# yesint/molar

Measured on AMD Instinct MI355X. Metric: frames/sec + Matom-pairs/sec, 1M-atom PBC neighbor search + RMSD fit, higher is better.
Workload: dtype f32; 1 GPU; 1M-atom synthetic triclinic box A, per frame: PBC neighbour search rc=1.2 nm (ordered pair list in HBM) + Kabsch RMSD fit/COM/gyration of a 100k-atom selection; natoms=1000000, selection_atoms=100000, frames_per_gpu=1451, parallelism=frames sharded over 1 rank(s), no data-path collective, streams_per_gpu=2, measure_overlapped_with_search=True

## Files before the change

molar_amd/csrc/pair_kernels.hpp:

```cpp
#pragma once

#include "boxmath.hpp"
#include "common.hpp"

namespace mh {
namespace pairk {

enum { MODE_COUNT = 0, MODE_FILL = 1, MODE_HIST = 2 };

#ifndef MH_COUNT_WPE
#define MH_COUNT_WPE 6
#endif
#ifndef MH_FILL_WPE
#define MH_FILL_WPE 8
#endif
#ifndef MH_WPB
#define MH_WPB 1
#endif
constexpr int waves_per_block(int mode) { return mode == MODE_HIST ? 4 : MH_WPB; }
constexpr int KREG = 8;
constexpr int FIFO_CAP = 128;
#ifndef MOLAR_HIP_NO_WIDE_FLUSH
#define MOLAR_HIP_WIDE_FLUSH 1
#endif
constexpr int FIFO_WIDE = 256;
constexpr uint32_t XCD_RUN = 128;
constexpr float F32_EPS = 1.1920929e-07f;
constexpr bool MASKED_COUNT_SORTED = true;

static __constant__ uint8_t MASKS[14][6] = {
    {0, 0, 0, 0, 0, 0},
    {0, 0, 0, 1, 0, 0}, {0, 0, 0, 0, 1, 0}, {0, 0, 0, 0, 0, 1},
    {0, 0, 0, 1, 1, 0}, {0, 0, 0, 1, 0, 1}, {0, 0, 0, 0, 1, 1},
    {0, 0, 0, 1, 1, 1},
    {1, 0, 0, 0, 1, 0}, {1, 0, 0, 0, 0, 1}, {0, 1, 0, 0, 0, 1},
    {1, 1, 0, 0, 0, 1}, {1, 0, 1, 0, 1, 0}, {0, 1, 1, 1, 0, 0},
};


typedef float v4f_t __attribute__((ext_vector_type(4)));
__device__ __forceinline__ float4 gload4(const float4 *p, size_t i) {
    const v4f_t v = ((const __attribute__((address_space(1))) v4f_t *)p)[i];
    return make_float4(v.x, v.y, v.z, v.w);
}
__device__ __forceinline__ uint32_t gload_u32(const uint32_t *p, size_t i) {
    return ((const __attribute__((address_space(1))) uint32_t *)p)[i];
}
__device__ __forceinline__ void gstore_u32(uint32_t *p, size_t i, uint32_t v) {
    ((__attribute__((address_space(1))) uint32_t *)p)[i] = v;
}
__device__ __forceinline__ float uniform_f32(float v) { return __uint_as_float(__builtin_amdgcn_readfirstlane(__float_as_uint(v))); }
__device__ __forceinline__ float4 lload4(const float4 *p, uint32_t i) {
    const v4f_t v = ((const __attribute__((address_space(3))) v4f_t *)p)[i];
    return make_float4(v.x, v.y, v.z, v.w);
}

struct SearchParams {
    const float4 *sa;
    const float4 *sb;
    const uint32_t *csa;
    const uint32_t *csb;
    const float *vdwa;
    const float *vdwb;
    const float4 *aabb_b;
    const float4 *perm_b;
    const float4 *chunk_aabb_b;
    const uint4 *h16_b;
    const float4 *cell_org_b;
    uint32_t mfma_count;
    const struct TaskDesc *task_desc;
    uint32_t *maskbuf;
    const unsigned long long *task_moff;
    unsigned long long mask_cap_units;
    unsigned long long out_cap;
    uint32_t dx, dy, dz;
    uint32_t pbc;
    uint32_t use_box;
    uint32_t nblocks;
    uint32_t wrap_kind;
    uint32_t prune_wrapped;
    float prune_limit2;
    uint32_t approx_wrapped;
    float band_lo, band_hi;
    uint32_t hist_nbins;
    float hist_min, hist_max;
    unsigned long long *hist_bins;
    unsigned long long *hist_total;
    const float *hist_edges;
    float hist_scale;
    uint32_t hist_lean;
    const uint32_t *hist_nslots;
#ifdef MOLAR_HIP_DEBUG_KNOBS
    uint32_t debug_skip;
    unsigned long long *dbg;
#endif
    float cutoff2;
    uint64_t ntasks;
    molar_hip_box box;
    alignas(16) float shifts4[96];
    uint32_t hist_big;
};

struct TaskDesc {
    uint32_t a0, n1, b0, n2, cb, flags, pad0, pad1;
};

struct SlotDesc {
    uint32_t a0, n1, b0, n2;
// ... 120 lines not shown
    if (WK == WK_DIAG) {
        sx = M[0] * fx;
        sy = M[4] * fy;
        sz = M[8] * fz;
    } else if (WK == WK_UPPER) {
        sx = (M[0] * fx + M[3] * fy) + M[6] * fz;
        sy = M[4] * fy + M[7] * fz;
        sz = M[8] * fz;
    } else {
        sx = (M[0] * fx + M[3] * fy) + M[6] * fz;
        sy = (M[1] * fx + M[4] * fy) + M[7] * fz;
        sz = (M[2] * fx + M[5] * fy) + M[8] * fz;
    }
    v2f best2 = (sx * sx + sy * sy) + sz * sz;
    if (WK != WK_DIAG && B.nshift != 0 && wrap == MOLAR_HIP_PBC_FULL) {
        if (WIDE4) {
            for (int k = 0; k < B.nshift; k += 4) {
                float sh[12];
#pragma unroll
                for (int q = 0; q < 12; ++q) sh[q] = P.shifts4[3 * k + q];
#pragma unroll
                for (int q = 0; q < 4; ++q) {
                    const v2f cx = sx + sh[3 * q], cy = sy + sh[3 * q + 1], cz = sz + sh[3 * q + 2];
                    const v2f n2 = (cx * cx + cy * cy) + cz * cz;
                    best2.x = n2.x < best2.x ? n2.x : best2.x;
                    best2.y = n2.y < best2.y ? n2.y : best2.y;
                }
            }
        } else {
            for (int k = 0; k < B.nshift; ++k) {
                const v2f cx = sx + P.box.shifts[3 * k], cy = sy + P.box.shifts[3 * k + 1], cz = sz + P.box.shifts[3 * k + 2];
                const v2f n2 = (cx * cx + cy * cy) + cz * cz;
                best2.x = n2.x < best2.x ? n2.x : best2.x;
                best2.y = n2.y < best2.y ? n2.y : best2.y;
            }
        }
    }
    return best2;
}

struct Fifo {
    uint32_t *fi, *fj, *fd;
    uint32_t head, tail;
    uint32_t quota;
    uint64_t base;
    uint32_t room;
    bool has_pairs, has_dist;
    uint2 *pairs;
    float *dist;
    uint32_t *ids;
    uint32_t *hist;
    float hmin, hmax, hn;
    uint32_t recompute;
    const float4 *la;
    float4 *fq_store;
    float4 *fq;
    uint4 *lh;
    uint32_t wrap;
};

template <bool WIDE4 = false>
__device__ __forceinline__ float wrapped_d2_exact(const SearchParams &P, uint32_t wrap, float vx, float vy, float vz);

struct Hit {
    uint32_t i, j;
    float d2;
};
__device__ __forceinline__ Hit fifo_hit(const SearchParams &P, const Fifo &F, uint32_t s) {
    const uint32_t w = F.fd[s];
    if (F.recompute == 0u) return Hit{F.fi[s], F.fj[s], __uint_as_float(w)};
    float4 a, b;
    if (F.fq) {
        a = lload4(F.la, w);
        b = lload4(F.fq, s);
    } else {
        a = lload4(F.la, w >> 26);
        b = gload4(P.sb, w & 0x3FFFFFFu);
    }
    const float dx = b.x - a.x, dy = b.y - a.y, dz = b.z - a.z;
    const float d2 = F.recompute == 1u ? wrapped_d2_exact(P, F.wrap, dx, dy, dz) : (dx * dx + dy * dy) + dz * dz;
    return Hit{__float_as_uint(a.w), __float_as_uint(b.w), d2};
}

template <int KIND, int CAP = FIFO_CAP>
__device__ __forceinline__ void fifo_flush(const SearchParams &P, Fifo &F, uint32_t count, uint32_t lane) {
    if (lane < count && (F.hist || F.head + lane < F.room)) {
        const uint32_t s = (F.head + lane) & (CAP - 1);
        uint32_t pos = F.head;
#ifdef MOLAR_HIP_DEBUG_KNOBS
        if (P.debug_skip & 32u) pos &= 63u;
#endif
        if (KIND == MOLAR_HIP_SEARCH_WITHIN) {
            __builtin_nontemporal_store(F.fi[s], &F.ids[pos]);
        } else if (F.hist) {
            const float d = __builtin_sqrtf(fifo_hit(P, F, s).d2);
            float fb = __builtin_floorf(F.hn * (d - F.hmin) / (F.hmax - F.hmin));
            if (fb != fb) fb = 0.0f;
            if (fb >= 0.0f && fb < F.hn) atomicAdd(&F.hist[(uint32_t)fb], 1u);
        } else {
            const Hit h = fifo_hit(P, F, s);
#ifdef MOLAR_HIP_DEBUG_KNOBS
            const float dist = __builtin_sqrtf(h.d2);
            const bool wr = (P.debug_skip & 16u) ? dist == -1.0f : true;
            if (F.has_pairs && wr) __builtin_nontemporal_store(((unsigned long long)h.j << 32) | h.i, reinterpret_cast<unsigned long long *>(&F.pairs[pos]));
            if (F.has_dist && wr) __builtin_nontemporal_store(dist, &F.dist[pos]);
#else
            if (F.has_pairs) __builtin_nontemporal_store(((unsigned long long)h.j << 32) | h.i, reinterpret_cast<unsigned long long *>(&F.pairs[pos]));
            if (F.has_dist) __builtin_nontemporal_store(__builtin_sqrtf(h.d2), &F.dist[pos]);
#endif
        }
    }
    F.head += count;
}

template <int KIND>
__device__ __forceinline__ void fifo_drain(const SearchParams &P, Fifo &F, uint32_t lane) {
    __builtin_amdgcn_wave_barrier();
    do {
        fifo_flush<KIND>(P, F, F.quota, lane);
        F.quota = 64u;
    } while (F.tail - F.head >= 64u);
}

template <int KIND>
__device__ __forceinline__ void fifo_flush_wide(const SearchParams &P, Fifo &F, uint32_t lane) {
    typedef uint32_t u4_t __attribute__((ext_vector_type(4)));
    typedef float f2_t __attribute__((ext_vector_type(2)));
    const uint32_t e = F.head + 2u * lane;
    if (e + 1u < F.room) {
        const uint32_t s0 = e & (FIFO_WIDE - 1), s1 = (e + 1u) & (FIFO_WIDE - 1);
        const u4_t pr = {F.fi[s0], F.fj[s0], F.fi[s1], F.fj[s1]};
        const f2_t ds = {__builtin_sqrtf(__uint_as_float(F.fd[s0])), __builtin_sqrtf(__uint_as_float(F.fd[s1]))};
        uint32_t at = F.head + lane;
        bool wr = true;
#ifdef MOLAR_HIP_DEBUG_KNOBS
        if (P.debug_skip & 16u) wr = ds.x == -1.0f;
        if (P.debug_skip & 32u) at = (F.head & 127u) + lane;
#endif
        if (F.has_pairs && wr) __builtin_nontemporal_store(pr, reinterpret_cast<u4_t *>(&F.pairs[at]));
        if (F.has_dist && wr) __builtin_nontemporal_store(ds, reinterpret_cast<f2_t *>(&F.dist[at]));
    } else if (e < F.room) {
        const uint32_t s0 = e & (FIFO_WIDE - 1);
        if (F.has_pairs) __builtin_nontemporal_store(((unsigned long long)F.fj[s0] << 32) | F.fi[s0], reinterpret_cast<unsigned long long *>(&F.pairs[F.head + lane]));
        if (F.has_dist) __builtin_nontemporal_store(__builtin_sqrtf(__uint_as_float(F.fd[s0])), &F.dist[F.head + lane]);
    }
    F.head += 128u;
}

template <int KIND>
__device__ __forceinline__ void fifo_drain_wide(const SearchParams &P, Fifo &F, uint32_t lane) {
    __builtin_amdgcn_wave_barrier();
    do {
        if (F.hist) {
            fifo_flush<KIND, FIFO_WIDE>(P, F, 64u, lane);
            fifo_flush<KIND, FIFO_WIDE>(P, F, 64u, lane);
        } else if (F.quota != 128u) {
            uint32_t left = F.quota;
            while (left) {
                const uint32_t c = left < 64u ? left : 64u;
                fifo_flush<KIND, FIFO_WIDE>(P, F, c, lane);
                left -= c;
            }
            F.quota = 128u;
        } else {
            fifo_flush_wide<KIND>(P, F, lane);
        }
    } while (F.tail - F.head >= 128u);
}

template <int KIND, bool FILL, int WK, bool TRI, int NCH, bool RUNTIME_NCH, bool WIDE4 = false>
__device__ __forceinline__ uint32_t run_task(const SearchParams &P, const Task &T, uint32_t i0, Fifo &F, uint32_t lane) {
    constexpr bool VDW = KIND == MOLAR_HIP_SEARCH_DOUBLE_VDW;
    constexpr bool WITHIN = KIND == MOLAR_HIP_SEARCH_WITHIN;
    constexpr bool STREAM = NCH == 0;
    constexpr int NPAIR = STREAM ? 1 : (NCH + 1) / 2;
    uint32_t total = 0;
    BoxRegs B;
    B.nshift = 0;
    if (WK != WK_NONE) {
#pragma unroll
        for (int k = 0; k < 9; ++k) {
            B.I[k] = P.box.inv[k];
            B.M[k] = P.box.m[k];
        }
        B.nshift = P.box.nshift;
    }
    const float cutoff2 = P.cutoff2;

    v2f bx[NPAIR], by[NPAIR], bz[NPAIR], bv[NPAIR];
    uint32_t bid[2 * NPAIR];
    auto load_b = [&](uint32_t jj, float &x, float &y, float &z, float &v, uint32_t &id) {
        float4 q = make_float4(0.f, 0.f, 0.f, 0.f);
        float rv = 0.f;
        if (jj < T.n2) {
            q = P.sb[T.b0 + jj];
            if (VDW) rv = P.vdwb[T.b0 + jj];
        }
        x = q.x; y = q.y; z = q.z; v = rv; id = __float_as_uint(q.w);
    };
    if (!STREAM) {
#pragma unroll
        for (int h = 0; h < NPAIR; ++h) {
            float x0, y0, z0, v0, x1, y1, z1, v1;
            load_b((uint32_t)(2 * h) * 64u + lane, x0, y0, z0, v0, bid[2 * h]);
            load_b((uint32_t)(2 * h + 1) * 64u + lane, x1, y1, z1, v1, bid[2 * h + 1]);
            bx[h] = v2f{x0, x1}; by[h] = v2f{y0, y1}; bz[h] = v2f{z0, z1}; bv[h] = v2f{v0, v1};
        }
    }
    const uint32_t nchunks = (T.n2 + 63u) >> 6;

    {
        float4 a = make_float4(0.f, 0.f, 0.f, 0.f);
        float ra = 0.f;
        if (i0 + lane < T.n1) {
            a = P.sa[T.a0 + i0 + lane];
            if (VDW) ra = P.vdwa[T.a0 + i0 + lane];
        }
        const uint32_t rows = T.n1 - i0 < T.rps ? T.n1 - i0 : T.rps;
        for (uint32_t r = 0; r < rows; ++r) {
            const uint32_t i = i0 + r;
            const float px = __int_as_float(__builtin_amdgcn_readlane(__float_as_int(a.x), r));
            const float py = __int_as_float(__builtin_amdgcn_readlane(__float_as_int(a.y), r));
            const float pz = __int_as_float(__builtin_amdgcn_readlane(__float_as_int(a.z), r));
            const uint32_t id_i = (uint32_t)__builtin_amdgcn_readlane(__float_as_int(a.w), r);
            float r1 = 0.f;
            if (VDW) r1 = __int_as_float(__builtin_amdgcn_readlane(__float_as_int(ra), r));
            bool found = false;
// ... 205 lines not shown

constexpr int MFMA_TILES = 10;

__device__ __forceinline__ float mfma_error_bound(float R, float c) {
    return 2.3841858e-07f * ((16.0f * R * R + 8.0f * c) + (4.0f * R + 1.0f));
}
__device__ __forceinline__ bool mfma_bound_usable(float R, float E, float c) {
    return R < 64.0f && E < 0.02f * c && (c + R * R) < 3.0e4f;
}

template <int KIND, bool TRI>
__device__ __forceinline__ uint32_t run_count_mfma(const SearchParams &P, const Task &T, uint32_t i0, float4 *la, uint4 *lh,
                                                   uint32_t lane, bool &done) {
    typedef uint32_t u4_t __attribute__((ext_vector_type(4)));
    typedef __attribute__((address_space(3))) u4_t lds_u4;
    typedef __attribute__((address_space(3))) uint32_t lds_u32;
    typedef __attribute__((address_space(1))) u4_t glb_u4;
    const float cutoff2 = P.cutoff2;
    const uint32_t rows = __builtin_amdgcn_readfirstlane(T.n1 - i0 < T.rps ? T.n1 - i0 : T.rps);
    const uint32_t kh = lane >> 5, cl = lane & 31u;
    const uint32_t nct = (T.n2 + 31u) >> 5;
    float4 a = make_float4(0.f, 0.f, 0.f, 0.f);
    if (lane < rows) a = gload4(P.sa, T.a0 + i0 + lane);
    const float4 org = gload4(P.cell_org_b, T.cb);
    bool need = lane < rows;
    if (!TRI) {
        const float4 blo = gload4(P.aabb_b, 2 * T.cb), bhi = gload4(P.aabb_b, 2 * T.cb + 1);
        need = need && !(aabb_d2(a.x, a.y, a.z, blo.x, blo.y, blo.z, bhi.x, bhi.y, bhi.z) > cutoff2);
    }
    const unsigned long long live = __builtin_amdgcn_ballot_w64(need);
    const uint32_t nlive = TRI ? rows : (uint32_t)__popcll(live);
    if (!TRI && nlive == 0u) return 0u;
    const uint32_t rank = TRI ? lane : __builtin_amdgcn_mbcnt_hi((uint32_t)(live >> 32), __builtin_amdgcn_mbcnt_lo((uint32_t)live, 0u));
    u4_t bq[MFMA_TILES];
#pragma unroll
    for (int t = 0; t < MFMA_TILES; ++t) {
        const uint32_t col = (uint32_t)t * 32u + cl;
        if (32u * (uint32_t)(t + 1) <= T.n2) {
            bq[t] = ((const glb_u4 *)P.h16_b)[T.b0 + col];
        } else {
            bq[t] = u4_t{0u, 0u, 0u, 0x00007BFFu};
            if (col < T.n2) bq[t] = ((const glb_u4 *)P.h16_b)[T.b0 + col];
        }
    }
    if (TRI || need) la[rank] = a;
    const float r0 = a.x - org.x, r1 = a.y - org.y, r2 = a.z - org.z;
    float ra2 = need ? (r0 * r0 + r1 * r1) + r2 * r2 : 0.0f;
    const bool fin = ra2 == ra2;
    for (int off = 32; off > 0; off >>= 1) ra2 = fmaxf(ra2, __shfl_xor(ra2, off, 64));
    const float R = 1.0001f * __builtin_sqrtf(ra2) + org.w;
    const float E = uniform_f32(mfma_error_bound(R, cutoff2));
    if (__builtin_amdgcn_ballot_w64(!fin) != 0ull || !mfma_bound_usable(R, E, cutoff2)) {
        done = false;
        return 0u;
    }
    {
        u4_t k0 = {0u, 0u, 0u, 0x00007BFFu}, k1 = {0u, 0u, 0u, 0x3C003C00u};
        if (!TRI) {
            ((lds_u4 *)lh)[2u * lane] = k0;
            ((lds_u4 *)lh)[2u * lane + 1u] = k1;
            __builtin_amdgcn_wave_barrier();
        }
        if (need) {
            const _Float16 h0 = (_Float16)r0, h1 = (_Float16)r1, h2 = (_Float16)r2;
            const _Float16 l0 = (_Float16)(r0 - (float)h0), l1 = (_Float16)(r1 - (float)h1), l2 = (_Float16)(r2 - (float)h2);
            const float e0 = (float)h0 + (float)l0, e1 = (float)h1 + (float)l1, e2 = (float)h2 + (float)l2;
            const float na = ((e0 * e0 + e1 * e1) + e2 * e2) - cutoff2;
            const _Float16 nh = (_Float16)na, nl = (_Float16)(na - (float)nh);
            const _Float16 m2 = (_Float16)-2.0f;
            const _Float16 g0 = m2 * h0, g1 = m2 * h1, g2 = m2 * h2, s0 = m2 * l0, s1 = m2 * l1, s2 = m2 * l2;
            k0 = u4_t{pack_h2(g0, g1), pack_h2(g2, g0), pack_h2(g1, g2), pack_h2(nh, nl)};
            k1 = u4_t{pack_h2(s0, s1), pack_h2(s2, s0), pack_h2(s1, s2), 0x3C003C00u};
        }
        if (TRI || need) {
            ((lds_u4 *)lh)[2u * rank] = k0;
            ((lds_u4 *)lh)[2u * rank + 1u] = k1;
        }
    }
    __builtin_amdgcn_wave_barrier();
    const u4_t a0q = ((const lds_u4 *)lh)[2u * cl + kh], a1q = ((const lds_u4 *)lh)[2u * (32u + cl) + kh];
    const v8h_t A0 = __builtin_bit_cast(v8h_t, a0q), A1 = __builtin_bit_cast(v8h_t, a1q);
    __builtin_amdgcn_wave_barrier();
    lds_u32 *todo = (lds_u32 *)lh;
    uint32_t ntodo = 0;
    uint32_t cnt = 0;
#pragma unroll
    for (int t = 0; t < MFMA_TILES; ++t) {
        if ((uint32_t)t < nct) {
            u4_t bt = bq[t];
            if (kh == 0u) bt.w = 0x3C003C00u;
            const v8h_t B = __builtin_bit_cast(v8h_t, bt);
#pragma unroll
            for (int rt = 0; rt < 2; ++rt) {
                bool diag = false;
                if (32u * (uint32_t)rt >= nlive) continue;
                if (TRI) {
                    const uint32_t row0 = i0 + 32u * (uint32_t)rt;
                    if (32u * (uint32_t)t + 31u <= row0) continue;
                    diag = 32u * (uint32_t)t <= row0 + 31u;
                }
                v16f_t acc = {0.f, 0.f, 0.f, 0.f, 0.f, 0.f, 0.f, 0.f, 0.f, 0.f, 0.f, 0.f, 0.f, 0.f, 0.f, 0.f};
                acc = __builtin_amdgcn_mfma_f32_32x32x16_f16(rt == 0 ? A0 : A1, B, acc, 0, 0, 0);
                if (TRI && diag) {
                    const int tv = (int)(32u * (uint32_t)t + cl) - (int)(i0 + 32u * (uint32_t)rt + 4u * kh);
#pragma unroll
                    for (int i = 0; i < 16; ++i) acc[i] = (tv > 8 * (i / 4) + (i % 4)) ? acc[i] : 1.0e30f;
                }
                uint32_t h = 0u;
                float m = INFINITY;
#pragma unroll
                for (int i = 0; i < 16; ++i) {
                    h = __builtin_amdgcn_alignbit(h, __float_as_uint(acc[i]), 31);
                    m = __builtin_fminf(m, __builtin_fabsf(acc[i]));
                }
                if (__builtin_amdgcn_ballot_w64(m < E) == 0ull) {
                    cnt += (uint32_t)__popc(h);
                } else {
                    if (lane == 0) todo[ntodo] = (uint32_t)(2 * t + rt);
                    ++ntodo;
                }
            }
        }
    }
    if (ntodo) {
        __builtin_amdgcn_wave_barrier();
        for (uint32_t q = 0; q < ntodo; ++q) {
            const uint32_t id = __builtin_amdgcn_readfirstlane(todo[q]);
            const uint32_t ct = id >> 1, rt = id & 1u;
            const uint32_t col = ct * 32u + cl;
            float4 b = make_float4(3.0e38f, 3.0e38f, 3.0e38f, 0.f);
            if (col < T.n2) b = gload4(P.sb, T.b0 + col);
            for (uint32_t r = 0; r < 16u; ++r) {
                const uint32_t row = 32u * rt + 16u * kh + r;
                const float4 p = lload4(la, row);
                const float dx = b.x - p.x, dy = b.y - p.y, dz = b.z - p.z;
                const float d2 = (dx * dx + dy * dy) + dz * dz;
                cnt += (row < nlive && (!TRI || col > i0 + row) && d2 <= cutoff2) ? 1u : 0u;
            }
        }
    }
    for (int off = 32; off > 0; off >>= 1) cnt += __shfl_xor(cnt, off, 64);
    return cnt;
}

template <int KIND>
__device__ __forceinline__ bool run_count_mfma_wrapped(const SearchParams &P, const Task &T, uint32_t i0, float4 *la, uint4 *lh,
                                                       uint32_t lane, uint32_t *mwords, uint32_t &count_out) {
    typedef uint32_t u4_t __attribute__((ext_vector_type(4)));
    typedef __attribute__((address_space(3))) u4_t lds_u4;
    typedef __attribute__((address_space(3))) uint32_t lds_u32;
    typedef __attribute__((address_space(1))) u4_t glb_u4;
    const float cutoff2 = P.cutoff2;
    const uint32_t rows = __builtin_amdgcn_readfirstlane(T.n1 - i0 < 64u ? T.n1 - i0 : 64u);
    const uint32_t kh = lane >> 5, cl = lane & 31u;
    const uint32_t nct = (T.n2 + 31u) >> 5, nch = (T.n2 + 63u) >> 6;
    float Sx = 0.f, Sy = 0.f, Sz = 0.f;
    for (int d = 0; d < 3; ++d) {
        if (!((T.wrap >> d) & 1u)) continue;
        const float sgn = ((T.wrap_b >> d) & 1u) ? 1.0f : -1.0f;
        Sx += sgn * P.box.m[3 * d];
        Sy += sgn * P.box.m[3 * d + 1];
        Sz += sgn * P.box.m[3 * d + 2];
    }
    float4 a = make_float4(0.f, 0.f, 0.f, 0.f);
    if (lane < rows) a = gload4(P.sa, T.a0 + i0 + lane);
    const float4 org = gload4(P.cell_org_b, T.cb);
    const float4 blo = gload4(P.aabb_b, 2 * T.cb), bhi = gload4(P.aabb_b, 2 * T.cb + 1);
    const bool need = lane < rows && !(aabb_d2(a.x - Sx, a.y - Sy, a.z - Sz, blo.x, blo.y, blo.z, bhi.x, bhi.y, bhi.z) > P.prune_limit2);
    const unsigned long long live = __builtin_amdgcn_ballot_w64(need);
    const uint32_t nlive = (uint32_t)__popcll(live);
    if (nlive == 0u) {
        count_out = 0u;
        return true;
    }
    const uint32_t rank = __builtin_amdgcn_mbcnt_hi((uint32_t)(live >> 32), __builtin_amdgcn_mbcnt_lo((uint32_t)live, 0u));
    const float r0 = (a.x - Sx) - org.x, r1 = (a.y - Sy) - org.y, r2 = (a.z - Sz) - org.z;
    float ra2 = need ? (r0 * r0 + r1 * r1) + r2 * r2 : 0.0f;
    float big = need ? fmaxf(fmaxf(fabsf(a.x), fabsf(a.y)), fabsf(a.z)) : 0.0f;
    const bool fin = ra2 == ra2;
    for (int off = 32; off > 0; off >>= 1) {
        ra2 = fmaxf(ra2, __shfl_xor(ra2, off, 64));
        big = fmaxf(big, __shfl_xor(big, off, 64));
    }
    const float R = 1.0001f * __builtin_sqrtf(ra2) + org.w;
    const float rc = __builtin_sqrtf(P.band_hi);
    const float L = (fmaxf(fmaxf(fabsf(org.x), fabsf(org.y)), fabsf(org.z)) + R) + (fmaxf(fmaxf(fabsf(Sx), fabsf(Sy)), fabsf(Sz)) + big);
    const float Em = mfma_error_bound(R, cutoff2);
    const float E = uniform_f32((P.band_hi - cutoff2) * 1.0001f + Em + 4.0f * (5.9604645e-08f * (2.0f * L + 2.0f * rc)) * rc);
    if (__builtin_amdgcn_ballot_w64(!fin || !(E == E) || !mfma_bound_usable(R, Em, cutoff2) || !(E < 0.06f * cutoff2)) != 0ull) return false;
    u4_t bq[MFMA_TILES];
#pragma unroll
    for (int t = 0; t < MFMA_TILES; ++t) {
        const uint32_t col = (uint32_t)t * 32u + cl;
        if (32u * (uint32_t)(t + 1) <= T.n2) {
            bq[t] = ((const glb_u4 *)P.h16_b)[T.b0 + col];
        } else {
            bq[t] = u4_t{0u, 0u, 0u, 0x00007BFFu};
            if (col < T.n2) bq[t] = ((const glb_u4 *)P.h16_b)[T.b0 + col];
        }
    }
    {
        ((lds_u4 *)lh)[2u * lane] = u4_t{0u, 0u, 0u, 0x00007BFFu};
        ((lds_u4 *)lh)[2u * lane + 1u] = u4_t{0u, 0u, 0u, 0x3C003C00u};
        __builtin_amdgcn_wave_barrier();
        if (need) {
            const _Float16 h0 = (_Float16)r0, h1 = (_Float16)r1, h2 = (_Float16)r2;
            const _Float16 l0 = (_Float16)(r0 - (float)h0), l1 = (_Float16)(r1 - (float)h1), l2 = (_Float16)(r2 - (float)h2);
            const float e0 = (float)h0 + (float)l0, e1 = (float)h1 + (float)l1, e2 = (float)h2 + (float)l2;
            const float na = ((e0 * e0 + e1 * e1) + e2 * e2) - cutoff2;
            const _Float16 nh = (_Float16)na, nl = (_Float16)(na - (float)nh);
            const _Float16 m2 = (_Float16)-2.0f;
            const _Float16 g0 = m2 * h0, g1 = m2 * h1, g2 = m2 * h2, s0 = m2 * l0, s1 = m2 * l1, s2 = m2 * l2;
            ((lds_u4 *)lh)[2u * rank] = u4_t{pack_h2(g0, g1), pack_h2(g2, g0), pack_h2(g1, g2), pack_h2(nh, nl)};
            ((lds_u4 *)lh)[2u * rank + 1u] = u4_t{pack_h2(s0, s1), pack_h2(s2, s0), pack_h2(s1, s2), 0x3C003C00u};
            la[rank] = a;
        }
    }
    __builtin_amdgcn_wave_barrier();
    const u4_t a0q = ((const lds_u4 *)lh)[2u * cl + kh], a1q = ((const lds_u4 *)lh)[2u * (32u + cl) + kh];
    const v8h_t A0 = __builtin_bit_cast(v8h_t, a0q), A1 = __builtin_bit_cast(v8h_t, a1q);
    __builtin_amdgcn_wave_barrier();
    lds_u32 *todo = (lds_u32 *)lh;
    constexpr uint32_t TODO_CAP = 512u;
// ... 104 lines not shown
                q = gload4(P.sb, T.b0 + jj);
                if (WRAPPED) { q.x += Sx; q.y += Sy; q.z += Sz; }
            }
            bx[k] = q.x; by[k] = q.y; bz[k] = q.z; bid[k] = __float_as_uint(q.w);
        }
    }
    const float cutoff2 = P.cutoff2;
    const float band_lo = P.band_lo, band_hi = P.band_hi;
    const uint32_t rows = __builtin_amdgcn_readfirstlane(T.n1 - i0 < T.rps ? T.n1 - i0 : T.rps);
    unsigned long long live;
    {
        float4 a = make_float4(0.f, 0.f, 0.f, 0.f);
        if (lane < rows) a = gload4(P.sa, T.a0 + i0 + lane);
        la[lane] = a;
        const float4 lo = gload4(P.aabb_b, 2 * T.cb), hi = gload4(P.aabb_b, 2 * T.cb + 1);
        bool need = true;
        if (TRI) {
        } else if (!WRAPPED) {
            need = !(aabb_d2(a.x, a.y, a.z, lo.x, lo.y, lo.z, hi.x, hi.y, hi.z) > cutoff2);
        } else if (approx) {
            need = !(aabb_d2(a.x - Sx, a.y - Sy, a.z - Sz, lo.x, lo.y, lo.z, hi.x, hi.y, hi.z) > P.prune_limit2);
        }
        live = __builtin_amdgcn_ballot_w64(lane < rows && need);
    }
    __builtin_amdgcn_wave_barrier();
    uint32_t total = 0;

    if (REPLAY) {
        if (!mwords) return 0u;
        F.recompute = WRAPPED ? 1u : 2u;
        F.la = la;
        F.wrap = T.wrap;
        F.fq = F.fq_store;
        float4 q[NCH];
#pragma unroll
        for (int k = 0; k < NCH; ++k) {
            const uint32_t jj = (uint32_t)k * 64u + lane;
            q[k] = make_float4(0.f, 0.f, 0.f, 0.f);
            if (jj < T.n2) q[k] = gload4(P.sb, T.b0 + jj);
        }
        uint32_t w[NCH];
        uint32_t nrow = 0;
        while (live) {
            if ((nrow & 31u) == 0u) {
#pragma unroll
                for (int k = 0; k < NCH; ++k) w[k] = gload_u32(mwords, ((nrow >> 5) * NCH + k) * 64u + lane);
            }
            ++nrow;
            const uint32_t r = (uint32_t)__builtin_ctzll(live);
            live &= ~(1ull << r);
#pragma unroll
            for (int k = 0; k < NCH; ++k) {
                const bool hit = (int32_t)w[k] < 0;
                w[k] += w[k];
                const unsigned long long mask = __builtin_amdgcn_ballot_w64(hit);
                if (mask) {
                    const uint32_t cnt = (uint32_t)__popcll(mask);
                    if (hit) {
                        const uint32_t s = __builtin_amdgcn_mbcnt_hi((uint32_t)(mask >> 32),
                                                                     __builtin_amdgcn_mbcnt_lo((uint32_t)mask, F.tail)) &
                                           (FIFO_CAP - 1);
                        F.fq[s] = q[k];
                        F.fd[s] = r;
                    }
                    F.tail += cnt;
                    total += cnt;
                    if (F.tail - F.head >= 64u) fifo_drain<KIND>(P, F, lane);
                }
            }
        }
        if (F.tail != F.head) {
            __builtin_amdgcn_wave_barrier();
            fifo_flush<KIND>(P, F, F.tail - F.head, lane);
        }
        F.recompute = 0u;
        F.fq = nullptr;
        return total;
    }

#ifdef MOLAR_HIP_WIDE_FLUSH
    constexpr bool WIDE = FILL && !WRAPPED && KIND != MOLAR_HIP_SEARCH_WITHIN;
#else
    constexpr bool WIDE = false;
#endif
    if (FILL) {
        F.recompute = (WRAPPED && approx) ? 1u : 0u;
        F.la = la;
        F.wrap = T.wrap;
        if (WIDE && !F.hist) F.quota = 128u - ((uint32_t)F.base & 127u);
    }
    uint32_t acc = 0;
    uint32_t acc_hi = 0;
    uint32_t hw[NCH];
    uint32_t su = 0, mu = 0;
    uint32_t nrow = 0;
    if (MASKED) {
#pragma unroll
        for (int k = 0; k < NCH; ++k) hw[k] = 0u;
    }
    auto store_group = [&](uint32_t g, uint32_t n) {
#pragma unroll
        for (int k = 0; k < NCH; ++k) {
            acc += (uint32_t)__popc(hw[k]);
            if (mwords) gstore_u32(mwords, (g * NCH + k) * 64u + lane, hw[k] << (32u - n));
            hw[k] = 0u;
        }
    };
    auto exact_d2 = [&](const float4 &p, uint32_t jj) -> float {
        float4 q = make_float4(3.0e38f, 3.0e38f, 3.0e38f, 0.f);
        if (jj < T.n2) q = gload4(P.sb, T.b0 + jj);
        return wrapped_d2_exact(P, T.wrap, q.x - p.x, q.y - p.y, q.z - p.z);
    };
    while (live) {
        const uint32_t r = (uint32_t)__builtin_ctzll(live);
        live &= ~(1ull << r);
        const float4 p = lload4(la, r);
        const uint32_t id_i = __float_as_uint(p.w);
        const uint32_t i = i0 + r;
#pragma unroll
        for (int k = 0; k < NCH; ++k) {
            if (TRI && (uint32_t)k * 64u + 63u <= i) {
                if (MASKED && !FILL) hw[k] += hw[k];
                continue;
            }
            const uint32_t jj = (uint32_t)k * 64u + lane;
            const float dx = bx[k] - p.x, dy = by[k] - p.y, dz = bz[k] - p.z;
            float d2 = (dx * dx + dy * dy) + dz * dz;
            if (WRAPPED && !approx) d2 = wrapped_d2_exact<FILL && !MASKED>(P, T.wrap, dx, dy, dz);
            if (TRI && (uint32_t)k * 64u <= i) d2 = (jj > i) ? d2 : INFINITY;
            if (!FILL) {
                if (MASKED) {
                    if (WRAPPED && approx) {
                        unsigned long long scr;
                        asm volatile("v_cmp_gt_f32 vcc, %4, %3\n\t"
                                     "v_addc_co_u32 %0, %2, %0, %0, vcc\n\t"
                                     "v_addc_co_u32 %1, %2, %1, %1, vcc"
                                     : "+v"(hw[k]), "+v"(su), "=&s"(scr) : "v"(d2), "s"(band_lo) : "vcc");
                        asm volatile("v_cmp_ge_f32 vcc, %2, %1\n\tv_addc_co_u32 %0, vcc, %0, %0, vcc" : "+v"(mu) : "v"(d2), "s"(band_hi) : "vcc");
                    } else {
                        asm volatile("v_cmp_ge_f32 vcc, %2, %1\n\tv_addc_co_u32 %0, vcc, %0, %0, vcc" : "+v"(hw[k]) : "v"(d2), "s"(cutoff2) : "vcc");
                    }
                } else if (WRAPPED && approx) {
                    asm volatile("v_cmp_gt_f32 vcc, %2, %1\n\tv_addc_co_u32 %0, vcc, 0, %0, vcc" : "+v"(acc) : "v"(d2), "s"(band_lo) : "vcc");
                    asm volatile("v_cmp_ge_f32 vcc, %2, %1\n\tv_addc_co_u32 %0, vcc, 0, %0, vcc" : "+v"(acc_hi) : "v"(d2), "s"(band_hi) : "vcc");
                } else {
                    asm volatile("v_cmp_ge_f32 vcc, %2, %1\n\tv_addc_co_u32 %0, vcc, 0, %0, vcc" : "+v"(acc) : "v"(d2), "s"(cutoff2) : "vcc");
                }
            } else {
                bool hit;
                uint32_t third = __float_as_uint(d2);
                if (WRAPPED && approx) {
                    const bool sure = d2 < band_lo, maybe = d2 <= band_hi;
                    hit = sure;
                    if (__builtin_amdgcn_ballot_w64(maybe && !sure)) hit = sure || (maybe && exact_d2(p, jj) <= cutoff2);
                    third = (r << 26) | (T.b0 + jj);
                } else {
                    hit = d2 <= cutoff2;
                }
                const unsigned long long mask = __builtin_amdgcn_ballot_w64(hit);
                if (mask) {
                    const uint32_t cnt = (uint32_t)__popcll(mask);
                    if (hit) {
                        const uint32_t rank = __builtin_amdgcn_mbcnt_hi((uint32_t)(mask >> 32), __builtin_amdgcn_mbcnt_lo((uint32_t)mask, 0u));
                        const uint32_t off = ((rank + F.tail) << 2) & (((WIDE ? FIFO_WIDE : FIFO_CAP) - 1u) << 2);
                        typedef __attribute__((address_space(3))) uint32_t lds_u32;
                        *(lds_u32 *)((__attribute__((address_space(3))) char *)F.fi + off) = id_i;
                        *(lds_u32 *)((__attribute__((address_space(3))) char *)F.fj + off) = bid[k];
                        *(lds_u32 *)((__attribute__((address_space(3))) char *)F.fd + off) = third;
                    }
                    F.tail += cnt;
                    total += cnt;
                    if (WIDE) {
                        if (F.tail - F.head >= 128u) fifo_drain_wide<KIND>(P, F, lane);
                    } else if (F.tail - F.head >= 64u) fifo_drain<KIND>(P, F, lane);
                }
            }
        }
        if (!FILL && WRAPPED && approx) {
            bool any_amb;
            if (MASKED) {
                any_amb = __builtin_amdgcn_ballot_w64(((su ^ mu) & ((1u << NCH) - 1u)) != 0u) != 0ull;
            } else {
                any_amb = __builtin_amdgcn_ballot_w64(acc != acc_hi) != 0ull;
            }
            if (any_amb) {
#pragma unroll
                for (int k = 0; k < NCH; ++k) {
                    const float dx = bx[k] - p.x, dy = by[k] - p.y, dz = bz[k] - p.z;
                    const float d2 = (dx * dx + dy * dy) + dz * dz;
                    const bool amb = d2 <= band_hi && !(d2 < band_lo);
                    if (__builtin_amdgcn_ballot_w64(amb)) {
                        if (amb && exact_d2(p, (uint32_t)k * 64u + lane) <= cutoff2) {
                            if (MASKED) hw[k] |= 1u;
                            else acc += 1u;
                        }
                    }
                }
                acc_hi = acc;
            }
        }
        if (!FILL && MASKED) {
            if ((++nrow & 31u) == 0u) store_group((nrow >> 5) - 1u, 32u);
        }
    }
    if (!FILL) {
        if (MASKED && (nrow & 31u) != 0u) store_group(nrow >> 5, nrow & 31u);
        for (int off = 32; off > 0; off >>= 1) acc += __shfl_xor(acc, off, 64);
        total = acc;
    } else if (F.tail != F.head) {
        __builtin_amdgcn_wave_barrier();
        if (WIDE) {
            while (F.tail != F.head) {
                const uint32_t c = F.tail - F.head < 64u ? F.tail - F.head : 64u;
                fifo_flush<KIND, FIFO_WIDE>(P, F, c, lane);
            }
        } else {
            fifo_flush<KIND>(P, F, F.tail - F.head, lane);
        }
    }
    if (FILL) F.recompute = 0u;
    return total;
}

constexpr int KMAX_WIDE = 16;
constexpr int KMAX_HUGE = 32;
template <int KIND, bool FILL, int WK, bool MASKED, int KMAX = KREG>
__device__ __forceinline__ uint32_t run_task_nch(const SearchParams &P, const Task &T, uint32_t i0, Fifo &F, float4 *la,
                                                 uint32_t lane, uint32_t *mwords) {
    const uint32_t nchunks = (T.n2 + 63u) >> 6;
    if constexpr (KMAX > KMAX_WIDE) {
        if ((KIND == MOLAR_HIP_SEARCH_SINGLE || KIND == MOLAR_HIP_SEARCH_DOUBLE) && nchunks > (uint32_t)KREG && nchunks <= (uint32_t)KMAX) {
            constexpr bool WR = WK != WK_NONE;
            const bool tri = KIND == MOLAR_HIP_SEARCH_SINGLE && WK == WK_NONE && T.tri;
            if (!T.tri || tri) {
#define MH_HUGE_CASE(N)                                                                                              \
    if (nchunks <= (uint32_t)(N)) {                                                                                  \
        if (tri) {                                                                                                   \
            if constexpr (KIND == MOLAR_HIP_SEARCH_SINGLE && WK == WK_NONE)                                          \
                return run_fast<KIND, FILL, false, N, true, false>(P, T, i0, F, la, lane, nullptr);                  \
        }                                                                                                            \
        return run_fast<KIND, FILL, WR, N, false, false>(P, T, i0, F, la, lane, nullptr);                            \
    }
                MH_HUGE_CASE(16) MH_HUGE_CASE(20) MH_HUGE_CASE(24) MH_HUGE_CASE(28) MH_HUGE_CASE(32)
#undef MH_HUGE_CASE
            }
        }
    } else if constexpr (KMAX > KREG) {
        if ((KIND == MOLAR_HIP_SEARCH_SINGLE || KIND == MOLAR_HIP_SEARCH_DOUBLE) && nchunks > (uint32_t)KREG && nchunks <= (uint32_t)KMAX) {
            constexpr bool WR = WK != WK_NONE;
            const bool tri = KIND == MOLAR_HIP_SEARCH_SINGLE && WK == WK_NONE && T.tri;
            if (!T.tri || tri) {
// ... 74 lines not shown
                                                   unsigned long long *__restrict__ scan_state, uint64_t nstate,
                                                   SearchParams *__restrict__ params_dst) {
    const uint64_t t = (uint64_t)blockIdx.x * blockDim.x + threadIdx.x;
    if (t < nslot_cnt) slot_cnt[t] = 0u;
    if (t < nstate) scan_state[t] = 0ull;
    if (params_dst && blockIdx.x == 0) {
        const uint32_t *src = (const uint32_t *)__builtin_amdgcn_kernarg_segment_ptr();
        uint32_t *d = (uint32_t *)params_dst;
        for (uint32_t w = threadIdx.x; w < (uint32_t)(sizeof(SearchParams) / 4u); w += blockDim.x) d[w] = src[w];
    }
    if (t == P.ntasks) {
        task_nb[t] = 0u;
        task_mu[t] = 0u;
    }
    if (t >= P.ntasks) return;
    const Task T = decode_task<KIND, false>(P, t);
    const uint32_t nb = T.valid ? (T.n1 + T.rps - 1u) / T.rps : 0u;
    task_nb[t] = nb;
    const uint32_t nch = (T.n2 + 63u) >> 6;
    task_mu[t] = (fast_kind && P.use_box && T.wrap != 0u && nch <= (uint32_t)KREG) ? nb * 2u * nch : 0u;
    TaskDesc d;
    d.a0 = T.a0; d.n1 = T.n1; d.b0 = T.b0; d.n2 = T.n2; d.cb = T.cb;
    d.flags = T.wrap | (T.tri ? 0x100u : 0u) | (T.valid ? 0x200u : 0u) | (T.wrap_b << 12) | (T.rps << 16);
    d.pad0 = d.pad1 = 0;
    task_desc[t] = d;
}

static __global__ void __launch_bounds__(256) slotmap_kernel(uint64_t ntasks, const uint32_t *__restrict__ task_first,
                                                      const TaskDesc *__restrict__ task_desc,
                                                      const unsigned long long *__restrict__ task_moff,
                                                      SlotDesc *__restrict__ slot_desc, uint64_t nslots_bound,
                                                      unsigned long long *__restrict__ sizes_host) {
    const uint64_t t = (uint64_t)blockIdx.x * blockDim.x + threadIdx.x;
    if (t == 0 && sizes_host) {
        sizes_host[1] = task_moff ? task_moff[ntasks] : 0ull;
        sizes_host[2] = task_first[ntasks];
    }
    if (t >= ntasks) {
        const uint64_t s = (uint64_t)task_first[ntasks] + (t - ntasks);
        if (s <= nslots_bound) {
            SlotDesc z;
            z.a0 = z.n1 = z.b0 = z.n2 = z.cb = z.flags = z.i0 = z.frame = 0u;
            z.moff = ~0ull >> 1;
            z.pad1 = 0ull;
            slot_desc[s] = z;
        }
        return;
    }
    const uint32_t s0 = task_first[t], s1 = task_first[t + 1];
    if (s1 == s0) return;
    const TaskDesc d = task_desc[t];
    const uint32_t rps = d.flags >> 16, nch = (d.n2 + 63u) >> 6;
    const unsigned long long m0 = task_moff ? task_moff[t] : (~0ull >> 1);
    for (uint32_t s = s0; s < s1; ++s) {
        SlotDesc o;
        o.a0 = d.a0; o.n1 = d.n1; o.b0 = d.b0; o.n2 = d.n2;
        o.cb = d.cb; o.flags = d.flags; o.i0 = (s - s0) * rps; o.frame = 0u;
        o.moff = task_moff ? m0 + (unsigned long long)(s - s0) * 2u * nch : m0;
        o.pad1 = 0ull;
        slot_desc[s] = o;
    }
}

template <int KIND>
__device__ __forceinline__ bool hist_lean_slot(const SearchParams &P, uint32_t flags, uint32_t n2) {
    if (KIND != MOLAR_HIP_SEARCH_SINGLE && KIND != MOLAR_HIP_SEARCH_DOUBLE) return false;
    if (((n2 + 63u) >> 6) > (uint32_t)KREG && !P.hist_big) return false;
    const uint32_t wrap = flags & 7u;
    if (!(P.use_box && wrap != 0u)) return true;
    if (flags & 0x100u) return false;
    return P.approx_wrapped != 0u && !(P.box.nshift != 0 && wrap == MOLAR_HIP_PBC_FULL);
}

template <int KIND, int MODE, int WPE = 0>
__global__ void __launch_bounds__(64 * waves_per_block(MODE))
__attribute__((amdgpu_waves_per_eu(WPE ? WPE : (MODE == MODE_HIST ? 4 : (MODE == MODE_COUNT ? MH_COUNT_WPE : MH_FILL_WPE))))) pair_kernel(const SearchParams *__restrict__ Pp,
                                                     const SlotDesc *__restrict__ slot_desc,
                                                     const uint32_t nslots_arg,
                                                     uint32_t *__restrict__ slot_cnt,
                                                     const unsigned long long *__restrict__ slot_base,
                                                     uint2 *__restrict__ out_pairs, float *__restrict__ out_dist,
                                                     uint32_t *__restrict__ out_ids) {
    constexpr int WAVES_PER_BLOCK = waves_per_block(MODE), BLOCK = 64 * WAVES_PER_BLOCK;
    constexpr int PLANE = MODE != MODE_COUNT ? FIFO_WIDE : FIFO_CAP;
    static_assert(FIFO_CAP * 16 <= 2 * FIFO_WIDE * 4, "the replay queue fits in two planes");
    __shared__ __attribute__((aligned(16))) uint32_t lds[WAVES_PER_BLOCK][3][PLANE];
    __shared__ float4 lds_a[WAVES_PER_BLOCK][64];
    __shared__ uint4 lds_h[MODE == MODE_COUNT ? WAVES_PER_BLOCK : 1][MODE == MODE_COUNT ? 128 : 1];
    constexpr bool FILL = MODE != MODE_COUNT;
    extern __shared__ uint32_t lds_hist[];
    const SearchParams &P0 = *Pp;
#ifdef MH_SLOT_LOOP
    uint32_t lane_var = threadIdx.x & 63u;
    const uint32_t &lane = lane_var;
#else
    const uint32_t lane = threadIdx.x & 63u;
#endif
    uint32_t nslots = nslots_arg;
    if (MODE == MODE_HIST && P0.hist_nslots) {
        const uint32_t real = __builtin_amdgcn_readfirstlane(P0.hist_nslots[0]);
        nslots = real < nslots_arg ? real : nslots_arg;
    }
    const uint32_t wave = WAVES_PER_BLOCK == 1 ? 0u : __builtin_amdgcn_readfirstlane(threadIdx.x >> 6);
    constexpr bool hist = MODE == MODE_HIST;
    if (hist) {
        for (uint32_t b = threadIdx.x; b < P0.hist_nbins; b += BLOCK) lds_hist[b] = 0u;
        __syncthreads();
    }
    unsigned long long wave_total = 0;
    auto process_slot = [&](uint32_t w) __attribute__((always_inline)) {
        uint32_t wr = w;
        {
            const uint32_t x = w & 7u, q = w >> 3;
            const uint32_t full = (nslots / (8u * XCD_RUN)) * (8u * XCD_RUN);
            if (w < full) wr = ((q / XCD_RUN) * 8u + x) * XCD_RUN + (q % XCD_RUN);
        }
        const uint32_t slot = nslots - 1u - wr;
        Task T;
        uint32_t i0;
        unsigned long long moff;
        uint32_t frame = 0u;
        {
            const uint4 lo = reinterpret_cast<const uint4 *>(slot_desc + slot)[0];
            const uint4 hi = reinterpret_cast<const uint4 *>(slot_desc + slot)[1];
            const uint2 mo = reinterpret_cast<const uint2 *>(slot_desc + slot)[4];
            const uint32_t fl = __builtin_amdgcn_readfirstlane(hi.y);
            if (!(fl & 0x200u)) return;
            if (MODE == MODE_HIST) frame = __builtin_amdgcn_readfirstlane(hi.w);
            T.a0 = __builtin_amdgcn_readfirstlane(lo.x);
            T.n1 = __builtin_amdgcn_readfirstlane(lo.y);
            T.b0 = __builtin_amdgcn_readfirstlane(lo.z);
            T.n2 = __builtin_amdgcn_readfirstlane(lo.w);
            T.cb = __builtin_amdgcn_readfirstlane(hi.x);
            i0 = __builtin_amdgcn_readfirstlane(hi.z);
            moff = ((unsigned long long)__builtin_amdgcn_readfirstlane(mo.y) << 32) | __builtin_amdgcn_readfirstlane(mo.x);
            T.wrap = fl & 7u;
            T.tri = (fl & 0x100u) != 0u;
            T.valid = true;
            T.wrap_b = (fl >> 12) & 7u;
            T.rps = fl >> 16;
        }
        const SearchParams &P = MODE == MODE_HIST ? Pp[frame] : P0;
        Fifo F;
        F.fi = lds[wave][0];
        F.fj = lds[wave][1];
        F.fd = lds[wave][2];
        F.head = F.tail = 0;
        F.quota = 64u;
        F.has_pairs = out_pairs != nullptr;
        F.has_dist = out_dist != nullptr;
        F.pairs = nullptr;
        F.dist = nullptr;
        F.ids = nullptr;
        F.base = 0;
        F.room = 0xFFFFFFFFu;
        F.hist = hist ? lds_hist : nullptr;
        F.recompute = 0u;
        F.la = lds_a[wave];
        F.fq = nullptr;
        F.fq_store = MODE == MODE_FILL ? reinterpret_cast<float4 *>(lds[wave][0]) : nullptr;
        F.lh = MODE == MODE_COUNT ? lds_h[wave] : nullptr;
        F.wrap = 0;
        F.hmin = P.hist_min;
        F.hmax = P.hist_max;
        F.hn = (float)P.hist_nbins;
        if (FILL && !hist) {
            F.base = slot_base[slot];
            F.quota = 64u - ((uint32_t)F.base & 63u);
// ... 106 lines not shown
```

Baseline: 749.4 frames/s.

## Recount ambiguous MFMA tiles per lane, add non-wrapping FIFO, correctly-rounded fast sqrt

In the MFMA count path, ambiguous tiles are no longer recounted whole. Each lane records a bitmask of the individual entries that fall inside the error band. Those entries are recomputed exactly in a parallel pass across lanes, with a fallback when the todo list overflows. The wide FIFO gains a slack region so LDS writes skip the modulo wrap, and overflowing entries are copied back to the front. sqrt of hit distances now uses the hardware approximate sqrt plus an FMA-based correction to keep rounding exact, falling back to the full sqrt for tiny inputs. The changes add LDS use and code complexity.

```diff
diff --git a/molar_amd/csrc/pair_kernels.hpp b/molar_amd/csrc/pair_kernels.hpp
--- a/molar_amd/csrc/pair_kernels.hpp
+++ b/molar_amd/csrc/pair_kernels.hpp
@@ -24,6 +24,7 @@
 #define MOLAR_HIP_WIDE_FLUSH 1
 #endif
 constexpr int FIFO_WIDE = 256;
+constexpr int FIFO_SLACK = 64;
 constexpr uint32_t XCD_RUN = 128;
 constexpr float F32_EPS = 1.1920929e-07f;
 constexpr bool MASKED_COUNT_SORTED = true;
@@ -310,6 +311,24 @@
     return Hit{__float_as_uint(a.w), __float_as_uint(b.w), d2};
 }
 
+__device__ __forceinline__ bool sqrt_hit_tiny(float d2) { return __builtin_amdgcn_ballot_w64(d2 < 0x1p-96f) != 0ull; }
+__device__ __forceinline__ float sqrt_rn_normal(float d2) {
+    const float s = __builtin_amdgcn_sqrtf(d2);
+    const float dn = __uint_as_float(__float_as_uint(s) - 1u), up = __uint_as_float(__float_as_uint(s) + 1u);
+    const float vp = __builtin_fmaf(-dn, s, d2), vs = __builtin_fmaf(-up, s, d2);
+    float r = vp <= 0.0f ? dn : s;
+    r = vs > 0.0f ? up : r;
+    return r;
+}
+__device__ __forceinline__ float sqrt_rn_hit(float d2) {
+#ifdef MH_PLAIN_SQRT
+    return __builtin_sqrtf(d2);
+#else
+    if (sqrt_hit_tiny(d2)) return __builtin_sqrtf(d2);
+    return sqrt_rn_normal(d2);
+#endif
+}
+
 template <int KIND, int CAP = FIFO_CAP>
 __device__ __forceinline__ void fifo_flush(const SearchParams &P, Fifo &F, uint32_t count, uint32_t lane) {
     if (lane < count && (F.hist || F.head + lane < F.room)) {
@@ -328,13 +347,13 @@
         } else {
             const Hit h = fifo_hit(P, F, s);
 #ifdef MOLAR_HIP_DEBUG_KNOBS
-            const float dist = __builtin_sqrtf(h.d2);
+            const float dist = sqrt_rn_hit(h.d2);
             const bool wr = (P.debug_skip & 16u) ? dist == -1.0f : true;
             if (F.has_pairs && wr) __builtin_nontemporal_store(((unsigned long long)h.j << 32) | h.i, reinterpret_cast<unsigned long long *>(&F.pairs[pos]));
             if (F.has_dist && wr) __builtin_nontemporal_store(dist, &F.dist[pos]);
 #else
             if (F.has_pairs) __builtin_nontemporal_store(((unsigned long long)h.j << 32) | h.i, reinterpret_cast<unsigned long long *>(&F.pairs[pos]));
-            if (F.has_dist) __builtin_nontemporal_store(__builtin_sqrtf(h.d2), &F.dist[pos]);
+            if (F.has_dist) __builtin_nontemporal_store(sqrt_rn_hit(h.d2), &F.dist[pos]);
 #endif
         }
     }
@@ -358,7 +377,15 @@
     if (e + 1u < F.room) {
         const uint32_t s0 = e & (FIFO_WIDE - 1), s1 = (e + 1u) & (FIFO_WIDE - 1);
         const u4_t pr = {F.fi[s0], F.fj[s0], F.fi[s1], F.fj[s1]};
-        const f2_t ds = {__builtin_sqrtf(__uint_as_float(F.fd[s0])), __builtin_sqrtf(__uint_as_float(F.fd[s1]))};
+        const float q0 = __uint_as_float(F.fd[s0]), q1 = __uint_as_float(F.fd[s1]);
+        f2_t ds;
+#ifdef MH_PLAIN_SQRT
+        const bool tiny = true;
+#else
+        const bool tiny = sqrt_hit_tiny(__builtin_fminf(q0, q1));
+#endif
+        if (tiny) ds = f2_t{__builtin_sqrtf(q0), __builtin_sqrtf(q1)};
+        else ds = f2_t{sqrt_rn_normal(q0), sqrt_rn_normal(q1)};
         uint32_t at = F.head + lane;
         bool wr = true;
 #ifdef MOLAR_HIP_DEBUG_KNOBS
@@ -370,7 +397,7 @@
     } else if (e < F.room) {
         const uint32_t s0 = e & (FIFO_WIDE - 1);
         if (F.has_pairs) __builtin_nontemporal_store(((unsigned long long)F.fj[s0] << 32) | F.fi[s0], reinterpret_cast<unsigned long long *>(&F.pairs[F.head + lane]));
-        if (F.has_dist) __builtin_nontemporal_store(__builtin_sqrtf(__uint_as_float(F.fd[s0])), &F.dist[F.head + lane]);
+        if (F.has_dist) __builtin_nontemporal_store(sqrt_rn_hit(__uint_as_float(F.fd[s0])), &F.dist[F.head + lane]);
     }
     F.head += 128u;
 }
@@ -742,6 +769,7 @@
     const v8h_t A0 = __builtin_bit_cast(v8h_t, a0q), A1 = __builtin_bit_cast(v8h_t, a1q);
     __builtin_amdgcn_wave_barrier();
     lds_u32 *todo = (lds_u32 *)lh;
+    [[maybe_unused]] constexpr uint32_t TODO_CAP = 512u;
     uint32_t ntodo = 0;
     uint32_t cnt = 0;
 #pragma unroll
@@ -776,12 +804,46 @@
                 if (__builtin_amdgcn_ballot_w64(m < E) == 0ull) {
                     cnt += (uint32_t)__popc(h);
                 } else {
+#ifdef MH_BLOCK_RECOUNT
                     if (lane == 0) todo[ntodo] = (uint32_t)(2 * t + rt);
                     ++ntodo;
-                }
-            }
-        }
-    }
+#else
+                    uint32_t u = 0u;
+#pragma unroll
+                    for (int i = 0; i < 16; ++i) u = 2u * u + (__builtin_fabsf(acc[i]) < E ? 1u : 0u);
+                    cnt += (uint32_t)__popc(h & ~u);
+                    const unsigned long long um = __builtin_amdgcn_ballot_w64(u != 0u);
+                    const uint32_t at = __builtin_amdgcn_mbcnt_hi((uint32_t)(um >> 32), __builtin_amdgcn_mbcnt_lo((uint32_t)um, ntodo));
+                    if (u != 0u && at < TODO_CAP) todo[at] = ((uint32_t)(2 * t + rt) << 22) | (lane << 16) | u;
+                    ntodo += (uint32_t)__popcll(um);
+#endif
+                }
+            }
+        }
+    }
+#ifndef MH_BLOCK_RECOUNT
+    if (ntodo > TODO_CAP) {
+        done = false;
+        return 0u;
+    }
+    if (ntodo) {
+        __builtin_amdgcn_wave_barrier();
+        for (uint32_t q = lane; q < ntodo; q += 64u) {
+            const uint32_t e = todo[q];
+            const uint32_t rt = (e >> 22) & 1u, col = (e >> 23) * 32u + ((e >> 16) & 31u), row0 = 32u * rt + 4u * ((e >> 21) & 1u);
+            float4 b = make_float4(3.0e38f, 3.0e38f, 3.0e38f, 0.f);
+            if (col < T.n2) b = gload4(P.sb, T.b0 + col);
+            for (uint32_t u = e & 0xFFFFu; u != 0u; u &= u - 1u) {
+                const uint32_t i = 15u - (uint32_t)__builtin_ctz(u);
+                const uint32_t row = row0 + 8u * (i >> 2) + (i & 3u);
+                const float4 p = lload4(la, row);
+                const float dx = b.x - p.x, dy = b.y - p.y, dz = b.z - p.z;
+                const float d2 = (dx * dx + dy * dy) + dz * dz;
+                cnt += (row < nlive && (!TRI || col > i0 + row) && d2 <= cutoff2) ? 1u : 0u;
+            }
+        }
+    }
+#else
     if (ntodo) {
         __builtin_amdgcn_wave_barrier();
         for (uint32_t q = 0; q < ntodo; ++q) {
@@ -799,6 +861,7 @@
             }
         }
     }
+#endif
     for (int off = 32; off > 0; off >>= 1) cnt += __shfl_xor(cnt, off, 64);
     return cnt;
 }
@@ -1069,6 +1132,11 @@
     constexpr bool WIDE = FILL && !WRAPPED && KIND != MOLAR_HIP_SEARCH_WITHIN;
 #else
     constexpr bool WIDE = false;
+#endif
+#ifdef MH_RING_WRAP
+    constexpr bool WIDE_NOWRAP = false;
+#else
+    constexpr bool WIDE_NOWRAP = WIDE;
 #endif
     if (FILL) {
         F.recompute = (WRAPPED && approx) ? 1u : 0u;
@@ -1149,11 +1217,23 @@
                     const uint32_t cnt = (uint32_t)__popcll(mask);
                     if (hit) {
                         const uint32_t rank = __builtin_amdgcn_mbcnt_hi((uint32_t)(mask >> 32), __builtin_amdgcn_mbcnt_lo((uint32_t)mask, 0u));
-                        const uint32_t off = ((rank + F.tail) << 2) & (((WIDE ? FIFO_WIDE : FIFO_CAP) - 1u) << 2);
+                        const uint32_t off = WIDE_NOWRAP ? (rank + (F.tail & (FIFO_WIDE - 1u))) << 2
+                                                         : ((rank + F.tail) << 2) & (((WIDE ? FIFO_WIDE : FIFO_CAP) - 1u) << 2);
                         typedef __attribute__((address_space(3))) uint32_t lds_u32;
                         *(lds_u32 *)((__attribute__((address_space(3))) char *)F.fi + off) = id_i;
                         *(lds_u32 *)((__attribute__((address_space(3))) char *)F.fj + off) = bid[k];
                         *(lds_u32 *)((__attribute__((address_space(3))) char *)F.fd + off) = third;
+                    }
+                    if (WIDE_NOWRAP) {
+                        const uint32_t end = (F.tail & (FIFO_WIDE - 1u)) + cnt;
+                        if (end > (uint32_t)FIFO_WIDE) {
+                            __builtin_amdgcn_wave_barrier();
+                            if (lane < end - (uint32_t)FIFO_WIDE) {
+                                F.fi[lane] = F.fi[FIFO_WIDE + lane];
+                                F.fj[lane] = F.fj[FIFO_WIDE + lane];
+                                F.fd[lane] = F.fd[FIFO_WIDE + lane];
+                            }
+                        }
                     }
                     F.tail += cnt;
                     total += cnt;
@@ -1394,8 +1474,8 @@
                                                      uint2 *__restrict__ out_pairs, float *__restrict__ out_dist,
                                                      uint32_t *__restrict__ out_ids) {
     constexpr int WAVES_PER_BLOCK = waves_per_block(MODE), BLOCK = 64 * WAVES_PER_BLOCK;
-    constexpr int PLANE = MODE != MODE_COUNT ? FIFO_WIDE : FIFO_CAP;
-    static_assert(FIFO_CAP * 16 <= 2 * FIFO_WIDE * 4, "the replay queue fits in two planes");
+    constexpr int PLANE = MODE != MODE_COUNT ? FIFO_WIDE + FIFO_SLACK : FIFO_CAP;
+    static_assert(MODE == MODE_COUNT || FIFO_CAP * 16 <= 2 * PLANE * 4,"the replay queue fits in two planes");
     __shared__ __attribute__((aligned(16))) uint32_t lds[WAVES_PER_BLOCK][3][PLANE];
     __shared__ float4 lds_a[WAVES_PER_BLOCK][64];
     __shared__ uint4 lds_h[MODE == MODE_COUNT ? WAVES_PER_BLOCK : 1][MODE == MODE_COUNT ? 128 : 1];
```

New measurement: 666.0 frames/s. 0.889x the previous value.
